# mir-group/allegro

Measured on NVIDIA H100. Metric: atom-steps/sec (energy+forces), higher is better.
Workload: dtype f32

## Files before the change

allegro_b200/_lib.py:

```python
from __future__ import annotations

import ctypes as C
import os
from typing import Optional, Sequence

import torch

from . import build as _build

AB2_F64, AB2_F32, AB2_BF16 = 0, 1, 2
ACT_NONE, ACT_SILU, ACT_MUL_DSILU = 0, 1, 2
EPI_NONE, EPI_MUL_DSILU = 0, 1
NL_SILU, NL_MISH, NL_GELU = 1, 2, 3
NOT_ELIGIBLE = -1
MAX_SEG = 4

DTYPE_ENUM = {torch.float64: AB2_F64, torch.float32: AB2_F32, torch.bfloat16: AB2_BF16}
ACC_DTYPE = {torch.float64: torch.float64, torch.float32: torch.float32, torch.bfloat16: torch.float32}

_LIB: Optional[C.CDLL] = None

_vp, _i64, _i32, _dbl = C.c_void_p, C.c_int64, C.c_int, C.c_double

_SIGNATURES = {
# ... 12 lines not shown
    "ab2_linear_packed_bytes": ([_i32, _i32, _i32], C.c_int64),
    "ab2_linear_pack": ([_i32, _i32, _i32, _vp, _vp, _vp], C.c_int),
    "ab2_mlp2_readout": ([_i32, _i32, _i64, _i32, _i32, _i32, _i32, _vp, _i64, _vp, _i64, _vp, _i64, _vp, _i64, _vp, _i64, _vp, _i64, _vp, _vp, _vp], C.c_int),
    "ab2_mlp2": ([_i32, _i32, _i64, _i32, _i32, _i32, _i32, _vp, _vp, _vp, _vp, _vp, _vp, _vp, _i64, _i32, _vp, _vp, _vp, _vp, _vp], C.c_int),
    "ab2_mlp2_nl": ([_i32, _i32, _i64, _i32, _i32, _i32, _i32, _vp, _vp, _vp, _vp, _vp, _vp, _vp, _i64, _i32, _vp, _vp, _vp, _vp, _vp, _i32], C.c_int),
    "ab2_mlp2_readout_nl": ([_i32, _i32, _i64, _i32, _i32, _i32, _i32, _vp, _i64, _vp, _i64, _vp, _i64, _vp, _i64, _vp, _i64, _vp, _i64, _vp, _vp, _vp, _i32],
                            C.c_int),
    "ab2_env_sum": ([_i32, _i32, _i64, _i32, _vp, _vp, _vp, _i64, _dbl, _vp, _vp], C.c_int),
    "ab2_env_bwd": ([_i32, _i32, _i64, _i64, _i32, _vp, _vp, _vp, _vp, _i64, _vp, _dbl, _vp, _i64, _vp, _vp], C.c_int),
    "ab2_tp_fwd": ([_i32, _i32, _i64, _i64, _i32, _i32, _i32, _i32, _vp, _vp, _vp, _vp, _vp, _vp, _i32, _vp, _vp, _i64, _vp, _vp], C.c_int),
    "ab2_tp_bwd": ([_i32, _i32, _i64, _i64, _i32, _i32, _i32, _i32, _vp, _vp, _vp, _vp, _vp, _vp, _i32, _vp, _vp, _i64, _vp, _vp, _vp, _i64, _vp, _vp, _vp], C.c_int),
    "ab2_tp_chain_fwd": ([_i32, _i32, _i64, _i64, _i32, _vp, _vp, _vp, _vp, _vp, _vp, _vp, _vp, _vp, _vp], C.c_int),
    "ab2_tp_chain_bwd": ([_i32, _i32, _i64, _i64, _i32, _vp, _vp, _vp, _vp, _vp, _vp, _vp, _vp, _vp, _vp, _vp, _vp, _vp, _vp], C.c_int),
    "ab2_edge_sum": ([_i32, _i64, _vp, _vp, _dbl, _vp, _vp], C.c_int),
    "ab2_edge_sum_bwd": ([_i32, _i64, _vp, _vp, _dbl, _vp, _vp], C.c_int),
    "ab2_force_scatter": ([_i32, _i64, _i64, _i64, _vp, _vp, _vp, _vp, _vp, _vp], C.c_int),
    "ab2_force_virial_scatter": ([_i32, _i64, _i64, _i64, _vp, _vp, _vp, _vp, _vp, _vp, _vp, _vp], C.c_int),
    "ab2_transpose_ui": ([_i32, _i64, _i32, _i32, _vp, _vp, _i32, _vp], C.c_int),
    "ab2_edge_vec": ([_i32, _i32, _i64, _vp, _vp, _vp, _vp, _vp, _vp], C.c_int),
    "ab2_radial_fwd": ([_i32, _i64, _i32, _i32, _dbl, _vp, _vp, _vp, _vp, _vp, _i32, _vp, _vp, _vp, _vp, _vp, _vp], C.c_int),
    "ab2_radial_pq_fwd": ([_i32, _i64, _i32, _i32, _dbl, _vp, _vp, _vp, _vp, _vp, _i32, _vp, _vp, _vp, _vp], C.c_int),
    "ab2_radial_pq_bwd": ([_i32, _i64, _i32, _i32, _dbl, _vp, _vp, _vp, _vp, _vp, _i32, _vp, _vp, _vp, _vp, _vp, _vp], C.c_int),
    "ab2_radial_pq_bwd_nl": ([_i32, _i64, _i32, _i32, _dbl, _vp, _vp, _vp, _vp, _vp, _i32, _vp, _vp, _vp, _vp, _vp, _vp, _i32], C.c_int),
    "ab2_zbl": ([_i32, _i64, _i32, _dbl, _dbl, _vp, _vp, _vp, _vp, _vp, _vp, _vp, _vp, _vp], C.c_int),
    "ab2_p2p_mailbox_bytes": ([_i32, _i32], C.c_int64),
    "ab2_p2p_alloc": ([_i64, C.POINTER(C.c_void_p)], C.c_int),
    "ab2_p2p_free": ([_vp], C.c_int),
    "ab2_p2p_get_handle": ([_vp, _vp], C.c_int),
    "ab2_p2p_open_handle": ([_vp, C.POINTER(C.c_void_p)], C.c_int),
    "ab2_p2p_close_handle": ([_vp], C.c_int),
    "ab2_p2p_error": ([_vp, _i32, _i32, _vp], C.c_int),
    "ab2_p2p_begin": ([_vp, _vp], C.c_int),
    "ab2_p2p_push_rows": ([_i32, _i32, _i32, _vp, _vp, _i32, _dbl, _vp, _i32, _i32, _vp, _vp, _vp], C.c_int),
    "ab2_p2p_wait_unpack": ([_i32, _i32, _i32, _vp, _i32, _i32, _vp, _i32, _vp, _vp, _i32, _vp], C.c_int),
    "ab2_p2p_allreduce_energy": ([_vp, _i32, _i32, _i32, _vp, _vp, _vp, _vp, _vp], C.c_int),
    "ab2_p2p_mailbox_bytes_ex": ([_i32, _i32, _i32], C.c_int64),
    "ab2_p2p_push_rows_w": ([_i32, _i32, _vp, _vp, _i32, _vp, _i32, _i32, _vp, _vp, _vp], C.c_int),
    "ab2_p2p_wait_unpack_w": ([_i32, _i32, _vp, _i32, _i32, _vp, _i32, _vp, _vp, _vp, _vp], C.c_int),
    "ab2_p2p_allreduce_vec": ([_vp, _i32, _i32, _i32, _i32, _vp, _vp, _vp, _vp, _vp], C.c_int),
    "ab2_slab_plan_count": ([_i32, _i32, _i64, _vp, _vp, _vp, _i32, _i32, _dbl, _dbl, _dbl, _vp, _vp, _vp], C.c_int),
    "ab2_slab_plan_fill": ([_i64, _vp, _vp, _vp, _vp, _vp, _vp], C.c_int),
    "ab2_nl_bin": ([_i32, _i64, _vp, _vp, _vp, _vp, _vp, _dbl, _vp, _vp], C.c_int),
    "ab2_nl_count": ([_i32, _i64, _vp, _vp, _vp, _vp, _vp, _dbl, _vp, _vp, _vp, _vp], C.c_int),
    "ab2_nl_fill": ([_i32, _i64, _vp, _vp, _vp, _vp, _vp, _dbl, _vp, _vp, _vp, _vp, _vp, _vp], C.c_int),
    "ab2_nl_lattice_bin": ([_i32, _i64, _vp, _vp, _vp, _vp, _vp, _vp, _dbl, _vp, _vp], C.c_int),
    "ab2_nl_lattice_count": ([_i32, _i64, _vp, _vp, _vp, _vp, _vp, _vp, _dbl, _vp, _vp, _vp, _vp], C.c_int),
# ... 584 lines not shown
    counts = torch.empty(n_centres, dtype=torch.int32, device=pos.device)
    with _timed(name + "_count"):
        _check(count_fn(dt, n_centres, _ptr(pos), *geom, _ptr(cell_start), _ptr(order), _ptr(counts), _stream()))
    row_ptr = torch.zeros(n_centres + 1, dtype=torch.int32, device=pos.device)
    row_ptr[1:] = torch.cumsum(counts, 0).to(torch.int32)
    E = int(row_ptr[-1])
    nbr = torch.empty(E, dtype=torch.int32, device=pos.device)
    shift = torch.empty(E, 3, dtype=pos.dtype, device=pos.device)
    if E:
        with _timed(name + "_fill"):
            _check(fill_fn(dt, n_centres, _ptr(pos), *geom, _ptr(cell_start), _ptr(order), _ptr(row_ptr), _ptr(nbr), _ptr(shift), _stream()))
    return row_ptr, nbr, shift


def radial_pq_fwd(dtype, S: int, p_cut: float, vec, ctr, nbr, types, rmax_table, bessel_w, PQ) -> torch.Tensor:
    E = ctr.shape[0]
    out = torch.empty(E, S, dtype=dtype, device=vec.device)
    with _timed("radial_fwd"):
        _check(load().ab2_radial_pq_fwd(DTYPE_ENUM[dtype], E, S, bessel_w.numel(), float(p_cut), _ptr(vec), _ptr(ctr), _ptr(nbr), _ptr(types),
                                        _ptr(rmax_table), rmax_table.shape[0], _ptr(bessel_w), _ptr(_contig(PQ, "PQ")), _ptr(out), _stream()))
    return out


def radial_pq_bwd(dtype, S: int, p_cut: float, vec, ctr, nbr, types, rmax_table, bessel_w, PQ, g_out, aux, gvec, nonlin: int = NL_SILU):
    E = ctr.shape[0]
    args = (DTYPE_ENUM[dtype], E, S, bessel_w.numel(), float(p_cut), _ptr(vec), _ptr(ctr), _ptr(nbr), _ptr(types), _ptr(rmax_table),
            rmax_table.shape[0], _ptr(bessel_w), _ptr(_contig(PQ, "PQ")), _ptr(_contig(g_out, "g_out")),
            _ptr(_contig(aux, "aux")) if aux is not None else None, _ptr(gvec), _stream())
    with _timed("radial_bwd"):
        _check(load().ab2_radial_pq_bwd(*args) if nonlin == NL_SILU else load().ab2_radial_pq_bwd_nl(*args, nonlin))


def _slab_plan(mode: int, pos: torch.Tensor, image: Optional[torch.Tensor], box, rank: int, world: int, width: float, jump: float,
               r_list: float, n_lists: int):
    n = pos.shape[0]
    if n == 0:
        return [torch.empty(0, dtype=torch.int64, device=pos.device) for _ in range(n_lists)], 0
    nblk = (n + 255) // 256
    cls = torch.empty(n, dtype=torch.uint8, device=pos.device)
    counts = torch.empty(nblk, 4, dtype=torch.int32, device=pos.device)
    boxa = (C.c_double * 3)(*[float(b) for b in box])
    with _timed("slab_plan_count"):
        _check(load().ab2_slab_plan_count(DTYPE_ENUM[pos.dtype], mode, n, _ptr(_contig(pos, "pos")), _ptr(image), boxa, int(rank), int(world),
                                          float(width), float(jump), float(r_list), _ptr(cls), _ptr(counts), _stream()))
    incl = torch.cumsum(counts, 0, dtype=torch.int32)
    offsets = (incl - counts).contiguous()
    lists = [torch.empty(n, dtype=torch.int64, device=pos.device) for _ in range(n_lists)]
    ptrs = [_ptr(t) for t in lists] + [None] * (3 - n_lists)
# ... 82 lines not shown
```

allegro_b200/csrc/linear_tc.cu:

```cuda
#include <cuda.h>

#include <type_traits>

#include "common.cuh"

extern int g_ab2_opt_linear_tc;
extern int g_ab2_opt_linear_tma;
extern int g_ab2_opt_tc_debug;

namespace {

constexpr int BM = 128;
constexpr int KC = 32;
constexpr int NSTAGE = 4;
constexpr int RAW_STAGE = 256 * 4 * 16;
constexpr int EPI_LD = 40;
constexpr int NCONS = 8;
constexpr int EPI_BYTES = NCONS * 16 * EPI_LD * 4;
constexpr int STAGE_HALF = BM * KC * 2;
constexpr int NPROD = 8;
constexpr int NTHREADS = (NPROD + NCONS) * 32;
constexpr int MAX_W_BYTES = 128 * 1024;
constexpr int MAX_K = 512;
constexpr int MAX_N = 128;
constexpr int MAX_CHUNK = MAX_N / 32;
constexpr int TAIL_BARS = 2 * NSTAGE * 8, TAIL_CHUNK = MAX_CHUNK * 32, TAIL_KMAP = (MAX_K / 8) * 16;
constexpr int TAIL_BYTES = TAIL_BARS + TAIL_CHUNK + 2 * TAIL_KMAP;
// ... 835 lines not shown
    uint64_t* rbars = reinterpret_cast<uint64_t*>(reinterpret_cast<uint8_t*>(sKseg) + (MAX_K / 32) * 16);
    const uint32_t bar0 = smem_u32(bars), rbar0 = smem_u32(rbars);
    const int nkb = p.K / KC;

    if (threadIdx.x == 0) tma_init_bars(bar0, rbar0, WPG);
    if (threadIdx.x < MAX_K / 32) {
        sKseg[threadIdx.x] = tma_kseg_entry(p, threadIdx.x);
    } else if (threadIdx.x >= 64 && threadIdx.x < 64 + MAX_CHUNK) {
        sChunk[threadIdx.x - 64] = tc_chunk_info<TSrc>(p, (threadIdx.x - 64) * 32);
    }
    stage_w(sW, p.Wpacked, p.Wlo, w_half);
    fence_proxy_async();
    __syncthreads();
    TcCtx ctx;
    ctx.sW = sW; ctx.sA = sA; ctx.sEpi = sEpi; ctx.sChunk = sChunk; ctx.bar0 = bar0;
    ctx.nkb = nkb; ctx.stage_bytes = stage_bytes; ctx.w_half = w_half;
    const int64_t my_tiles = (p.num_tiles > blockIdx.x) ? (p.num_tiles - blockIdx.x + gridDim.x - 1) / gridDim.x : 0;
    const int64_t total = my_tiles * nkb;

    if (warp >= NPROD) {
        tc_consumer_role<TSrc, SPLIT, NCH, NL>(p, ctx, warp - NPROD, lane);
    } else {
        tma_converter_role<G, NL>(p, maps, NR, ctx, sRaw, sKseg, rbar0, total, warp, lane);
    }
}

constexpr int MLP2_MAX_H = 64;
constexpr int MLP2_CHUNK = 64;
constexpr int MLP2_MAX_CHUNKS = 4;
constexpr int MLP2_TAIL = TAIL_BARS + (1 + MLP2_MAX_CHUNKS) * TAIL_CHUNK + (MAX_K / 32) * 16 + 8 * 8;

struct Mlp2Params {
    TcParams s1;
    TcParams s2[MLP2_MAX_CHUNKS];
    int n0[MLP2_MAX_CHUNKS];
    int n2;
    int w2_npad;
    int backward;
    const float* pre;
    int64_t pre_ld;
    const float* gout1;
    int64_t gout1_ld;
    const float* w1row;
};

template <int NCH>
// ... 457 lines not shown
    return fn;
}

static bool tc_make_map(CUtensorMap* map, const void* ptr, int64_t ld, int width, int64_t M) {
    EncodeTiledFn fn = tc_encode_fn();
    if (!fn) return false;
    const cuuint64_t dims[2] = {(cuuint64_t)width, (cuuint64_t)M};
    const cuuint64_t strides[1] = {(cuuint64_t)ld * 4};
    const cuuint32_t box[2] = {(cuuint32_t)KC, (cuuint32_t)BM};
    const cuuint32_t estr[2] = {1, 1};
    return fn(map, CU_TENSOR_MAP_DATA_TYPE_FLOAT32, 2, const_cast<void*>(ptr), dims, strides, box, estr, CU_TENSOR_MAP_INTERLEAVE_NONE,
              CU_TENSOR_MAP_SWIZZLE_128B, CU_TENSOR_MAP_L2_PROMOTION_L2_128B, CU_TENSOR_MAP_FLOAT_OOB_FILL_NONE) == CUDA_SUCCESS;
}

template <typename F>
static int tc_with_nl(int nonlin, F&& f) {
    switch (nonlin) {
        case AB2_NL_MISH: return f(std::integral_constant<int, AB2_NL_MISH>{});
        case AB2_NL_GELU: return f(std::integral_constant<int, AB2_NL_GELU>{});
        default: return f(std::integral_constant<int, AB2_NL_SILU>{});
    }
}

static int tc_launch_tma(TcParams& p, int w_bytes, int stage_bytes, int max_smem, unsigned grid, cudaStream_t st, bool dry, int nonlin) {
    TmaMaps maps;
    memset(&maps, 0, sizeof(maps));
    if (!tc_encode_fn()) return -1;
    for (int s = 0; s < p.n_a && !dry; ++s) {
        if (!tc_make_map(&maps.a[s], p.a[s].ptr, p.a[s].ld, p.a[s].width, p.M)) return -1;
        if (p.a[s].aux && !tc_make_map(&maps.x[s], p.a[s].aux, p.a[s].aux_ld, p.a[s].width, p.M)) return -1;
    }
    const int raw_slot = TMA_BOX_BYTES * (p.has_aux ? 2 : 1);
    const int plans[6][3] = {{4, 8, 4}, {4, 4, 4}, {2, 4, 4}, {2, 2, 4}, {2, 4, 2}, {2, 2, 2}};
    int G = 0, NR = 0, nstage = 0;
    size_t smem = 0;
    for (int q = 0; q < 6 && !G; ++q) {
        const size_t need = 1024 + ((w_bytes + 127) & ~127) + (size_t)plans[q][2] * stage_bytes + EPI_BYTES + TAIL_BYTES +
                            (size_t)plans[q][1] * raw_slot;
        if (need <= (size_t)max_smem) { G = plans[q][0]; NR = plans[q][1]; nstage = plans[q][2]; smem = need; }
    }
    if (!G) return -1;
    if (dry) return 0;
    p.nstage = nstage;
    auto go = [&](auto kern) -> int {
        if (cudaFuncSetAttribute(kern, cudaFuncAttributeMaxDynamicSharedMemorySize, (int)smem) != cudaSuccess) {
            cudaGetLastError();
            return -1;
        }
        kern<<<grid, NTHREADS, smem, st>>>(p, maps, NR);
        return 0;
    };
    return tc_with_nl(nonlin, [&](auto nl) -> int {
        constexpr int NL = decltype(nl)::value;
        switch ((G == 4 ? 4 : 0) + p.Npad / 32) {
            case 1: return go(linear_tma_kernel<2, 1, NL>);
            case 2: return go(linear_tma_kernel<2, 2, NL>);
            case 3: return go(linear_tma_kernel<2, 3, NL>);
            case 4: return go(linear_tma_kernel<2, 4, NL>);
            case 5: return go(linear_tma_kernel<4, 1, NL>);
            case 6: return go(linear_tma_kernel<4, 2, NL>);
            case 7: return go(linear_tma_kernel<4, 3, NL>);
            case 8: return go(linear_tma_kernel<4, 4, NL>);
        }
        return -1;
// ... 112 lines not shown
        const int ns = (N - n0 < width) ? (N - n0) : width;
        void* so_ptr[AB2_MAX_SEG];
        int64_t so_ld[AB2_MAX_SEG];
        int32_t so_w[AB2_MAX_SEG], so_acc[AB2_MAX_SEG];
        int cnt = 0, seg_lo = 0;
        for (int s = 0; s < n_o; ++s) {
            const int seg_hi = seg_lo + o_width[s];
            const int a = n0 > seg_lo ? n0 : seg_lo, b = (n0 + ns) < seg_hi ? (n0 + ns) : seg_hi;
            if (a < b) {
                so_ptr[cnt] = reinterpret_cast<uint8_t*>(o_ptr[s]) + (size_t)(a - seg_lo) * esz;
                so_ld[cnt] = o_ld[s];
                so_w[cnt] = b - a;
                so_acc[cnt] = o_accum ? o_accum[s] : 0;
                ++cnt;
            }
            seg_lo = seg_hi;
        }
        const void* aux_s = aux ? reinterpret_cast<const uint8_t*>(aux) + (size_t)n0 * esz : nullptr;
        const int rc = tc_launch_slice(dtype, M, K, ns, n_a, a_ptr, a_ld, a_width, a_aux, a_aux_ld, act, hi + (size_t)n0 * K * 2,
                                       lo + (size_t)n0 * K * 2, cnt, so_ptr, so_ld, so_w, so_acc, epi, aux_s, aux_ld, st, nonlin);
        if (rc != 0) return n0 == 0 ? -1 : 1;
    }
    return 0;
}

extern "C" int ab2_mlp2_nl(int dtype, int backward, int64_t M, int K, int H, int N, int n_a, const void* const* a_ptr, const int64_t* a_ld,
                           const int32_t* a_width, const void* W1_packed, const void* W2_packed, const void* w1_row, void* pre, int64_t pre_ld,
                           int n_o, void* const* o_ptr, const int64_t* o_ld, const int32_t* o_width, const int32_t* o_accum, void* stream,
                           int nonlin) {
    AB2_CHECK_ARG(nonlin == AB2_NL_SILU || nonlin == AB2_NL_MISH || nonlin == AB2_NL_GELU, "nonlinearity");
    AB2_CHECK_ARG(n_a >= 1 && n_a <= AB2_MAX_SEG && n_o >= 1 && n_o <= AB2_MAX_SEG, "segment count");
    AB2_CHECK_ARG(K > 0 && H > 0 && N > 0 && pre && pre_ld >= H, "shape");
    int ks = 0, ns = 0;
    for (int s = 0; s < n_a; ++s) {
        AB2_CHECK_ARG(a_ptr[s] && a_width[s] > 0 && a_ld[s] >= a_width[s], "A segment");
        ks += a_width[s];
    }
    for (int s = 0; s < n_o; ++s) {
        AB2_CHECK_ARG(o_ptr[s] && o_width[s] > 0 && o_ld[s] >= o_width[s], "output segment");
        ns += o_width[s];
    }
    AB2_CHECK_ARG(ks == K, "A segment widths must sum to K");
    AB2_CHECK_ARG(ns == N, "output segment widths must sum to N");
    const bool rank1 = w1_row != nullptr;
    AB2_CHECK_ARG(!rank1 || (backward && K == 1 && n_a == 1), "rank-1 mode is the backward of a single output column");
    if (M == 0) return 0;
// ... 206 lines not shown
```

allegro_b200/csrc/radial.cu:

```cuda
#include "common.cuh"

#define AB2_MAX_BESSEL 16

template <typename T>
__device__ __forceinline__ T ab2_sin(T x);
template <>
__device__ __forceinline__ float ab2_sin<float>(float x) { return sinf(x); }
template <>
__device__ __forceinline__ double ab2_sin<double>(double x) { return sin(x); }
template <typename T>
__device__ __forceinline__ T ab2_cos(T x);
template <>
__device__ __forceinline__ float ab2_cos<float>(float x) { return cosf(x); }
template <>
__device__ __forceinline__ double ab2_cos<double>(double x) { return cos(x); }
__device__ __forceinline__ float ab2_pow(float x, float p) { return powf(x, p); }
__device__ __forceinline__ double ab2_pow(double x, double p) { return pow(x, p); }

template <typename TPos, typename TAcc>
__global__ void __launch_bounds__(256) edge_vec_kernel(int64_t E, const TPos* __restrict__ pos, const int32_t* __restrict__ ctr,
                                                       const int32_t* __restrict__ nbr, const TPos* __restrict__ shift,
                                                       TAcc* __restrict__ vec) {
    const int64_t z = (int64_t)blockIdx.x * 256 + threadIdx.x;
    if (z >= E) return;
    const int64_t i = ctr[z], j = nbr[z];
#pragma unroll
    for (int a = 0; a < 3; ++a) {
        TPos d = pos[j * 3 + a] - pos[i * 3 + a];
        if (shift) d += shift[z * 3 + a];
        vec[z * 3 + a] = (TAcc)d;
    }
}

template <typename TAcc, bool GRAD>
__device__ __forceinline__ void bessel_basis(TAcc x, TAcc p, int nb, const TAcc* __restrict__ bw, TAcc* B, TAcc* dB) {
    const TAcc PI = TAcc(3.14159265358979323846);
    if (x >= TAcc(1)) {
        for (int n = 0; n < nb; ++n) {
            B[n] = TAcc(0);
            if (GRAD) dB[n] = TAcc(0);
        }
        return;
    }
    const TAcc xp = ab2_pow(x, p);
    const TAcc a = (p + 1) * (p + 2) / 2, b = p * (p + 2), c = p * (p + 1) / 2;
    const TAcc f = TAcc(1) - a * xp + b * xp * x - c * xp * x * x;
    const TAcc df = GRAD ? (-a * p * xp / x + b * (p + 1) * xp - c * (p + 2) * xp * x) : TAcc(0);
    const TAcc inv = TAcc(1) / (PI * x);
    for (int n = 0; n < nb; ++n) {
        const TAcc arg = PI * bw[n] * x;
        const TAcc s = ab2_sin(arg) * inv;
        B[n] = s * f;
        if (GRAD) {
            const TAcc ds = (bw[n] * ab2_cos(arg) - s) / x;
            dB[n] = ds * f + s * df;
        }
    }
}

template <typename TAct, typename TAcc>
__global__ void __launch_bounds__(256) radial_fwd_kernel(int64_t E, int S_rc, int nb, TAcc p, const TAcc* __restrict__ vec,
                                                         const int32_t* __restrict__ ctr, const int32_t* __restrict__ nbr,
                                                         const int32_t* __restrict__ types, const TAcc* __restrict__ rmax_table,
                                                         int num_types, const TAcc* __restrict__ bw, const TAcc* __restrict__ Wb,
                                                         const TAcc* __restrict__ cemb, const TAcc* __restrict__ nemb,
                                                         TAct* __restrict__ e0) {
    __shared__ TAcc sB[AB2_MAX_BESSEL][256];
    __shared__ int s_tc[256], s_tn[256];
    const int t = threadIdx.x;
    const int64_t z0 = (int64_t)blockIdx.x * 256;
    {
        const int64_t z = z0 + t;
        TAcc B[AB2_MAX_BESSEL];
        int tc = 0, tn = 0;
        if (z < E) {
            const TAcc vx = vec[z * 3], vy = vec[z * 3 + 1], vz = vec[z * 3 + 2];
            const TAcc r = sqrt(vx * vx + vy * vy + vz * vz);
            tc = types[ctr[z]];
            tn = types[nbr[z]];
// ... 282 lines not shown
```

allegro_b200/nn/_pipeline.py:

```python
from __future__ import annotations

import math
from typing import Dict, List, Optional

import torch

from .. import _lib
from ..data import EdgeCSR
from ._mlp import PackedMLP


def _env_perm(U: int, n_ir: int, individual: bool = True) -> torch.Tensor:
    r = torch.arange(n_ir).view(-1, 1)
    u = torch.arange(U).view(1, -1)
    if not individual:
        return (u + 0 * r).reshape(-1)
    return (u * n_ir + r).reshape(-1)


class _Saved:
    __slots__ = ("csr", "vec", "Y", "w0", "omega", "V", "gamma", "pre_lat", "pre_read", "X", "fold", "chain")


_BAKED_TABLES = {}
# ... 303 lines not shown
        self.rmax_table = edge_norm.rmax_table.detach().to(device=device, dtype=acc).contiguous()
        self.bessel_w = radial.bessel_encode.bessel_weights.detach().reshape(-1).to(device=device, dtype=acc).contiguous()
        self.Wb = te.basis_linear.folded_weights()[0].to(device=device, dtype=acc).contiguous()
        self.cemb = te.center_embed.weight.detach().to(device=device, dtype=acc).contiguous()
        self.nemb = te.neighbor_embed.weight.detach().to(device=device, dtype=acc).contiguous()
        self.PQ, self.S_pq, self.fold_radial = None, 0, False
        nb = int(self.bessel_w.numel())
        import os as _os

        if nb == 8 and _os.environ.get("ALLEGRO_B200_RADIAL_PQ", "1") == "1":
            Wb64 = te.basis_linear.folded_weights()[0].detach().double().cpu()
            ce, ne = te.center_embed.weight.detach().double().cpu(), te.neighbor_embed.weight.detach().double().cpu()
            T = ce.shape[0]
            temb = torch.cat([ce.unsqueeze(1).expand(T, T, -1), ne.unsqueeze(0).expand(T, T, -1)], dim=-1)
            PQ0 = temb.reshape(T * T, 1, -1) * Wb64.unsqueeze(0)
            if self.mlp.is_two_layer_nonlinear and self.mlp.dims[1] <= 128 and _os.environ.get("ALLEGRO_B200_FOLD_RADIAL", "1") == "1":
                self.fold_radial = True
                PQ0 = PQ0 @ self.mlp.W64[0]
            if PQ0.shape[-1] <= 128:
                self.PQ = PQ0.to(device=device, dtype=acc).contiguous()
                self.S_pq = int(PQ0.shape[-1])
            else:
                self.fold_radial = False

    def forward(self, vec, csr: EdgeCSR, types_i32, outs):
        dt = self.dtype
        if self.kind == "spline":
            from ._spline import spline_forward

            t64 = types_i32.long()
            e0, sp_saved = spline_forward(vec, t64[csr.ctr.long()], t64[csr.nbr.long()], self.rmax64, self.sp_lower, self.sp_upper, self.sp_const,
                                          self.sp_w, self.num_types, dt)
            return ("spline", sp_saved, self.mlp.forward([e0], outs))
        if self.fold_radial:
            h = _lib.radial_pq_fwd(dt, self.S_pq, self.p, vec, csr.ctr, csr.nbr, types_i32, self.rmax_table, self.bessel_w, self.PQ)
            _lib.linear([h], self.mlp.W[1], outs, act=_lib.ACT_SILU, W_packed=self.mlp.Wp[1], **self.mlp.nl_kw)
            return ("pq_fold", None, [h])
        if self.PQ is not None:
            e0 = _lib.radial_pq_fwd(dt, self.S_pq, self.p, vec, csr.ctr, csr.nbr, types_i32, self.rmax_table, self.bessel_w, self.PQ)
        else:
            e0 = _lib.radial_fwd(dt, self.S_rc, self.p, vec, csr.ctr, csr.nbr, types_i32, self.rmax_table, self.bessel_w, self.Wb, self.cemb, self.nemb)
        return ("bessel", None, self.mlp.forward([e0], outs))

    def backward(self, saved, gouts, vec, csr: EdgeCSR, types_i32, gvec):
        kind, sp_saved, pre = saved
        dt = self.dtype
        E = vec.shape[0]
        if kind == "pq_fold":
            g_h = self.mlp.hidden_grad(gouts)
            _lib.radial_pq_bwd(dt, self.S_pq, self.p, vec, csr.ctr, csr.nbr, types_i32, self.rmax_table, self.bessel_w, self.PQ, g_h, pre[0], gvec,
                               **self.mlp.nl_kw)
            return
        g_e0 = torch.empty(E, self.S_rc, dtype=dt, device=vec.device)
        if self.mlp.is_two_layer_nonlinear:
            self.mlp.backward_plain(gouts, pre, [g_e0])
        else:
            self.mlp.backward(gouts, pre, [g_e0], [False])
        if kind == "spline":
            from ._spline import spline_backward

            gvec += spline_backward(sp_saved, g_e0, self.sp_w, self.num_types).to(gvec.dtype)
        elif self.PQ is not None:
            _lib.radial_pq_bwd(dt, self.S_pq, self.p, vec, csr.ctr, csr.nbr, types_i32, self.rmax_table, self.bessel_w, self.PQ, g_e0, None, gvec)
        else:
            _lib.radial_bwd(dt, self.S_rc, self.p, vec, csr.ctr, csr.nbr, types_i32, self.rmax_table, self.bessel_w, self.Wb, self.cemb, self.nemb, g_e0, gvec)


def energy_forces(core: "AllegroCore", up: UpstreamPack, csr: EdgeCSR, pos: torch.Tensor, types_i32: torch.Tensor,
                  shift_vec: Optional[torch.Tensor], gEi_scale: Optional[torch.Tensor], want_virial: bool = False, pair=None,
                  frame_ptr: Optional[torch.Tensor] = None, want_atomic_virial: bool = False):
    dt, acc = core.dtype, core.acc
# ... 65 lines not shown
```

include/allegro_b200.h:

```cpp
#ifndef ALLEGRO_B200_H
#define ALLEGRO_B200_H
#include <stdint.h>

#ifdef __cplusplus
extern "C" {
#endif

enum { AB2_F64 = 0, AB2_F32 = 1, AB2_BF16 = 2 };
enum { AB2_ACT_NONE = 0, AB2_ACT_SILU = 1, AB2_ACT_MUL_DSILU = 2 };
enum { AB2_EPI_NONE = 0, AB2_EPI_MUL_DSILU = 1 };
enum { AB2_NL_SILU = 1, AB2_NL_MISH = 2, AB2_NL_GELU = 3 };

#define AB2_MAX_SEG 4
#define AB2_MAX_LMAX 4

const char* ab2_last_error(void);
int ab2_version(void);
int ab2_device_ok(void);
int ab2_set_option(const char* key, int value);


int ab2_op_scatter_env(int dtype, int64_t E, int64_t row , double sf,
                       const void* x2, const int64_t* idxs, void* gamma, void* stream);

// ... 132 lines not shown
int ab2_nl_frames_fill(int pos_dtype, int64_t n, int64_t n_frames, const int32_t* frame_ptr, const void* pos,
                       const void* cell, const void* inv_cell, const int32_t* pbc, const int32_t* nimg, double r_max,
                       const int32_t* row_ptr, int32_t* nbr, void* shift, void* stream);

int64_t ab2_frame_scratch_elems(int64_t total, int64_t n_frames);
int ab2_frame_sum(int acc_dtype, int64_t n, int64_t n_frames, const int32_t* frame_ptr, const void* x, double* scratch,
                  int64_t scratch_elems, void* out, void* stream);
int ab2_frame_virial(int acc_dtype, int64_t E, int64_t n_frames, const int32_t* frame_ptr, const int32_t* row_ptr,
                     const void* vec, const void* gvec, double* scratch, int64_t scratch_elems, void* W, void* stream);
int ab2_frame_heat_current(int acc_dtype, int64_t n, int64_t n_frames, const int32_t* frame_ptr, const void* e_atom,
                           const void* vel, const void* W, double* scratch, int64_t scratch_elems, void* J, void* stream);

int ab2_radial_pq_fwd(int dtype, int64_t E, int S, int num_bessels, double p_cut, const void* vec,
                      const int32_t* ctr, const int32_t* nbr, const int32_t* types, const void* rmax_table,
                      int num_types, const void* bessel_w, const void* PQ, void* out, void* stream);
int ab2_radial_pq_bwd(int dtype, int64_t E, int S, int num_bessels, double p_cut, const void* vec,
                      const int32_t* ctr, const int32_t* nbr, const int32_t* types, const void* rmax_table,
                      int num_types, const void* bessel_w, const void* PQ, const void* g_out, const void* aux,
                      void* gvec, void* stream);
int ab2_radial_pq_bwd_nl(int dtype, int64_t E, int S, int num_bessels, double p_cut, const void* vec,
                         const int32_t* ctr, const int32_t* nbr, const int32_t* types, const void* rmax_table,
                         int num_types, const void* bessel_w, const void* PQ, const void* g_out, const void* aux,
                         void* gvec, void* stream, int nonlin);

int ab2_zbl(int acc_dtype, int64_t E, int num_types, double p_cut, double qq, const void* vec, const int32_t* ctr,
            const int32_t* nbr, const int32_t* types, const void* Z, const void* rmax_table, void* Ez, void* gvec,
            void* stream);


int64_t ab2_p2p_mailbox_bytes(int max_rows, int world);
int ab2_p2p_alloc(int64_t bytes, void** ptr);
int ab2_p2p_free(void* ptr);
int ab2_p2p_get_handle(void* ptr, void* handle64_host);
int ab2_p2p_open_handle(const void* handle64_host, void** ptr);
int ab2_p2p_close_handle(void* ptr);
int ab2_p2p_error(void* my_mailbox, int max_rows, int world, void* stream);
int ab2_p2p_begin(void* step_counter, void* stream);
int ab2_p2p_push_rows(int src_dtype, int kind, int side, const void* src, const int64_t* idx, int n, double shift_x,
                      void* peer_mailbox, int max_rows, int world, const void* step_counter, void* done_counter,
                      void* stream);
int ab2_p2p_wait_unpack(int dst_dtype, int kind, int side, void* my_mailbox, int max_rows, int world,
                        const void* step_counter, int n, void* dst, const int64_t* idx, int accumulate, void* stream);
int ab2_p2p_allreduce_energy(const void* e_local, int rank, int world, int max_rows, void* const* peers_dev,
                             void* my_mailbox, const void* step_counter, void* e_total, void* stream);

#define AB2_P2P_EXT_VIRIAL 1
// ... 22 lines not shown
```

Before: 3.466 million.

## Fuse radial MLP hidden-grad GEMM with radial basis adjoint in one TMA kernel

Adds a tensor-core TMA kernel that computes the output-layer gradient GEMM (gradient segments times packed W_out) and, in its epilogue, applies the activation derivative, contracts with the Bessel-basis derivative through PQ, and writes the edge-vector gradient. This replaces the separate hidden_grad GEMM plus radial_pq_bwd kernel for f32 with 8 Bessels and S of 32 or 64. The goal is to avoid materialising and re-reading the E x S hidden gradient and to save a launch. In exchange, the consumer warps' epilogue recomputes the Bessel basis and does per-row PQ gathers, which adds register pressure and shared-memory use. The bessel_basis helper moves into a shared header.

```diff
diff --git a/allegro_b200/_lib.py b/allegro_b200/_lib.py
--- a/allegro_b200/_lib.py
+++ b/allegro_b200/_lib.py
@@ -58,6 +58,9 @@
     "ab2_radial_pq_fwd": ([_i32, _i64, _i32, _i32, _dbl, _vp, _vp, _vp, _vp, _vp, _i32, _vp, _vp, _vp, _vp], C.c_int),
     "ab2_radial_pq_bwd": ([_i32, _i64, _i32, _i32, _dbl, _vp, _vp, _vp, _vp, _vp, _i32, _vp, _vp, _vp, _vp, _vp, _vp], C.c_int),
     "ab2_radial_pq_bwd_nl": ([_i32, _i64, _i32, _i32, _dbl, _vp, _vp, _vp, _vp, _vp, _i32, _vp, _vp, _vp, _vp, _vp, _vp, _i32], C.c_int),
+    "ab2_radial_pq_bwd_gemm_plan": ([_i32, _i32, _i32, _i32, _vp], C.c_int),
+    "ab2_radial_pq_bwd_gemm_nl": ([_i32, _i64, _i32, _i32, _dbl, _vp, _vp, _vp, _vp, _vp, _i32, _vp, _vp, _i32, _vp, _vp, _vp, _vp, _vp, _i64, _vp,
+                                   _vp, _i32], C.c_int),
     "ab2_zbl": ([_i32, _i64, _i32, _dbl, _dbl, _vp, _vp, _vp, _vp, _vp, _vp, _vp, _vp, _vp], C.c_int),
     "ab2_p2p_mailbox_bytes": ([_i32, _i32], C.c_int64),
     "ab2_p2p_alloc": ([_i64, C.POINTER(C.c_void_p)], C.c_int),
@@ -688,8 +691,30 @@
     return out
 
 
-def radial_pq_bwd(dtype, S: int, p_cut: float, vec, ctr, nbr, types, rmax_table, bessel_w, PQ, g_out, aux, gvec, nonlin: int = NL_SILU):
+def radial_pq_bwd_gemm_plan(dtype, S: int, num_bessels: int, seg_widths: Sequence[int]) -> bool:
+    w = (C.c_int32 * len(seg_widths))(*seg_widths)
+    return load().ab2_radial_pq_bwd_gemm_plan(DTYPE_ENUM[dtype], int(S), int(num_bessels), len(seg_widths), w) == 0
+
+
+def radial_pq_bwd(dtype, S: int, p_cut: float, vec, ctr, nbr, types, rmax_table, bessel_w, PQ, g_out, aux, gvec, nonlin: int = NL_SILU, *,
+                  W_out: Optional[torch.Tensor] = None, W_out_packed: Optional[torch.Tensor] = None):
     E = ctr.shape[0]
+    if W_out_packed is not None:
+        K, S_w = W_out.shape
+        assert S_w == S and aux is not None and aux.dtype == dtype and tuple(aux.shape) == (E, S)
+        aux, aux_ld = _row_strided(aux, "aux")
+        n = len(g_out)
+        g_ptr, g_ld, g_w = (C.c_void_p * n)(), (C.c_int64 * n)(), (C.c_int32 * n)()
+        for s, t in enumerate(g_out):
+            t, ld = _row_strided(t, f"gradient segment {s}")
+            assert t.dtype == dtype and t.shape[0] == E
+            g_ptr[s], g_ld[s], g_w[s] = _ptr(t).value, ld, t.shape[1]
+        assert sum(g_w) == K
+        with _timed("radial_bwd"):
+            _check(load().ab2_radial_pq_bwd_gemm_nl(DTYPE_ENUM[dtype], E, S, bessel_w.numel(), float(p_cut), _ptr(vec), _ptr(ctr), _ptr(nbr),
+                                                    _ptr(types), _ptr(rmax_table), rmax_table.shape[0], _ptr(bessel_w), _ptr(_contig(PQ, "PQ")),
+                                                    n, g_ptr, g_ld, g_w, _ptr(W_out_packed), _ptr(aux), aux_ld, _ptr(gvec), _stream(), nonlin))
+        return
     args = (DTYPE_ENUM[dtype], E, S, bessel_w.numel(), float(p_cut), _ptr(vec), _ptr(ctr), _ptr(nbr), _ptr(types), _ptr(rmax_table),
             rmax_table.shape[0], _ptr(bessel_w), _ptr(_contig(PQ, "PQ")), _ptr(_contig(g_out, "g_out")),
             _ptr(_contig(aux, "aux")) if aux is not None else None, _ptr(gvec), _stream())
diff --git a/allegro_b200/csrc/linear_tc.cu b/allegro_b200/csrc/linear_tc.cu
--- a/allegro_b200/csrc/linear_tc.cu
+++ b/allegro_b200/csrc/linear_tc.cu
@@ -3,6 +3,7 @@
 #include <type_traits>
 
 #include "common.cuh"
+#include "radial_basis.cuh"
 
 extern int g_ab2_opt_linear_tc;
 extern int g_ab2_opt_linear_tma;
@@ -884,6 +885,178 @@
         tc_consumer_role<TSrc, SPLIT, NCH, NL>(p, ctx, warp - NPROD, lane);
     } else {
         tma_converter_role<G, NL>(p, maps, NR, ctx, sRaw, sKseg, rbar0, total, warp, lane);
+    }
+}
+
+struct RadialAdj {
+    const float* vec;
+    const int32_t* ctr;
+    const int32_t* nbr;
+    const int32_t* types;
+    const float* rmax_table;
+    const float* bw;
+    const float* PQ;
+    const float* h;
+    float* gvec;
+    int64_t h_ld;
+    int num_types;
+    float p_cut;
+};
+
+constexpr int RADJ_LD = 16;
+
+__device__ __forceinline__ float2 ldg64_nc(const float* p) {
+    float2 v;
+    asm volatile("ld.global.nc.v2.f32 {%0, %1}, [%2];" : "=f"(v.x), "=f"(v.y) : "l"(p));
+    return v;
+}
+
+__device__ __forceinline__ int radj_rows(const TcParams& p, int64_t m_base) {
+    const int64_t left64 = p.M - m_base;
+    return left64 >= 16 ? 16 : (left64 > 0 ? (int)left64 : 0);
+}
+
+template <int NCH>
+__device__ __forceinline__ void radial_adjoint_prologue(const TcParams& p, const RadialAdj& ra, float* stg, float2 (&hv)[2][4 * NCH],
+                                                        int64_t m_base, int lane) {
+    const int rows_left = radj_rows(p, m_base);
+    if (rows_left == 0) return;
+    const int ra0 = lane >> 2, q = lane & 3;
+#pragma unroll
+    for (int hr = 0; hr < 2; ++hr) {
+        const int r = min(ra0 + 8 * hr, rows_left - 1);
+        const float* hz = ra.h + (m_base + r) * ra.h_ld + 2 * q;
+#pragma unroll
+        for (int j = 0; j < 4 * NCH; ++j) hv[hr][j] = ldg64_nc(hz + 8 * j);
+    }
+    const int row = lane & 15, half = lane >> 4;
+    float* s = stg + row * RADJ_LD;
+    float B[4], dB[4];
+    float vx = 0.f, vy = 0.f, vz = 0.f, den = 1.f, g0 = 0.f, g1 = 0.f, g2 = 0.f;
+    int pair = 0;
+    if (row < rows_left) {
+        const int64_t z = m_base + row;
+        vx = ra.vec[z * 3]; vy = ra.vec[z * 3 + 1]; vz = ra.vec[z * 3 + 2];
+        if (!half) { g0 = ra.gvec[z * 3]; g1 = ra.gvec[z * 3 + 1]; g2 = ra.gvec[z * 3 + 2]; }
+        const float r = sqrt(vx * vx + vy * vy + vz * vz);
+        pair = ra.types[ra.ctr[z]] * ra.num_types + ra.types[ra.nbr[z]];
+        const float rmax = ra.rmax_table[pair];
+        bessel_basis<float, true>(r / rmax, ra.p_cut, 4, ra.bw + 4 * half, B, dB);
+        den = rmax * r;
+    } else {
+#pragma unroll
+        for (int n = 0; n < 4; ++n) dB[n] = 0.f;
+    }
+#pragma unroll
+    for (int n = 0; n < 4; ++n) s[4 * half + n] = dB[n];
+    if (!half) {
+        s[8] = __int_as_float(pair); s[9] = den; s[10] = vx; s[11] = vy; s[12] = vz;
+        s[13] = g0; s[14] = g1; s[15] = g2;
+    }
+}
+
+template <int NCH, int NL>
+__device__ __forceinline__ void radial_adjoint_epilogue(const TcParams& p, const RadialAdj& ra, float* stg, const float (&acc)[16 * NCH],
+                                                        const float2 (&hv)[2][4 * NCH], int64_t m_base, int lane) {
+    constexpr int S = 32 * NCH;
+    const int rows_left = radj_rows(p, m_base);
+    if (rows_left == 0) return;
+    __syncwarp();
+    const int ra0 = lane >> 2, q = lane & 3;
+    const float* sa = stg + ra0 * RADJ_LD;
+    const float* sb = stg + (ra0 + 8) * RADJ_LD;
+    float dBa[8], dBb[8];
+#pragma unroll
+    for (int n = 0; n < 8; ++n) { dBa[n] = sa[n]; dBb[n] = sb[n]; }
+    const int pa = __float_as_int(sa[8]), pb = __float_as_int(sb[8]);
+    const float* ma = ra.PQ + (int64_t)pa * 8 * S + 2 * q;
+    const float* mb = ra.PQ + (int64_t)pb * 8 * S + 2 * q;
+    const bool same = pa == pb;
+    float ga = 0.f, gb = 0.f;
+#pragma unroll
+    for (int j = 0; j < 4 * NCH; ++j) {
+        float sa0 = 0.f, sa1 = 0.f, sb0 = 0.f, sb1 = 0.f;
+#pragma unroll
+        for (int n = 0; n < 8; ++n) {
+            const float2 wa = __ldg(reinterpret_cast<const float2*>(ma + n * S + 8 * j));
+            const float2 wb = same ? wa : __ldg(reinterpret_cast<const float2*>(mb + n * S + 8 * j));
+            sa0 += dBa[n] * wa.x;
+            sa1 += dBa[n] * wa.y;
+            sb0 += dBb[n] * wb.x;
+            sb1 += dBb[n] * wb.y;
+        }
+        float a0 = acc[4 * j], a1 = acc[4 * j + 1], b0 = acc[4 * j + 2], b1 = acc[4 * j + 3];
+        a0 *= dact_f<NL>(hv[0][j].x);
+        a1 *= dact_f<NL>(hv[0][j].y);
+        b0 *= dact_f<NL>(hv[1][j].x);
+        b1 *= dact_f<NL>(hv[1][j].y);
+        ga += a0 * sa0;
+        ga += a1 * sa1;
+        gb += b0 * sb0;
+        gb += b1 * sb1;
+    }
+    ga += __shfl_xor_sync(0xffffffffu, ga, 1);
+    ga += __shfl_xor_sync(0xffffffffu, ga, 2);
+    gb += __shfl_xor_sync(0xffffffffu, gb, 1);
+    gb += __shfl_xor_sync(0xffffffffu, gb, 2);
+    if (q < 2) {
+        const int r = ra0 + 8 * q;
+        if (r < rows_left) {
+            const float* s = q ? sb : sa;
+            const float f = (q ? gb : ga) / s[9];
+            float* gv = ra.gvec + (m_base + r) * 3;
+            gv[0] = s[13] + f * s[10];
+            gv[1] = s[14] + f * s[11];
+            gv[2] = s[15] + f * s[12];
+        }
+    }
+    __syncwarp();
+}
+
+template <int G, int NCH, int NL>
+__global__ void __launch_bounds__(NTHREADS, 1) radial_adjoint_tma_kernel(const TcParams p, const __grid_constant__ TmaMaps maps, int NR,
+                                                                       const RadialAdj ra) {
+    constexpr int WPG = NPROD / G;
+    extern __shared__ __align__(1024) uint8_t smem[];
+    const int warp = __shfl_sync(0xffffffffu, threadIdx.x >> 5, 0), lane = threadIdx.x & 31;
+    const int w_half = p.Npad * p.K * 2;
+    const int w_bytes = 2 * w_half;
+    const int stage_bytes = 2 * STAGE_HALF;
+    uint8_t* sRaw = smem + ((1024u - (smem_u32(smem) & 1023u)) & 1023u);
+    uint8_t* sW = sRaw + (size_t)NR * TMA_BOX_BYTES;
+    uint8_t* sA = sW + ((w_bytes + 127) & ~127);
+    float* sEpi = reinterpret_cast<float*>(sA + p.nstage * stage_bytes);
+    uint64_t* bars = reinterpret_cast<uint64_t*>(reinterpret_cast<uint8_t*>(sEpi) + EPI_BYTES);
+    int4* sKseg = reinterpret_cast<int4*>(reinterpret_cast<uint8_t*>(bars) + TAIL_BARS + TAIL_CHUNK);
+    uint64_t* rbars = reinterpret_cast<uint64_t*>(reinterpret_cast<uint8_t*>(sKseg) + (MAX_K / 32) * 16);
+    const uint32_t bar0 = smem_u32(bars), rbar0 = smem_u32(rbars);
+    const int nkb = p.K / KC;
+
+    if (threadIdx.x == 0) tma_init_bars(bar0, rbar0, WPG);
+    if (threadIdx.x < MAX_K / 32) sKseg[threadIdx.x] = tma_kseg_entry(p, threadIdx.x);
+    stage_w(sW, p.Wpacked, p.Wlo, w_half);
+    fence_proxy_async();
+    __syncthreads();
+    TcCtx ctx;
+    ctx.sW = sW; ctx.sA = sA; ctx.sEpi = sEpi; ctx.sChunk = nullptr; ctx.bar0 = bar0;
+    ctx.nkb = nkb; ctx.stage_bytes = stage_bytes; ctx.w_half = w_half;
+    const int64_t my_tiles = (p.num_tiles > blockIdx.x) ? (p.num_tiles - blockIdx.x + gridDim.x - 1) / gridDim.x : 0;
+
+    if (warp >= NPROD) {
+        const int cw = warp - NPROD, wg = cw >> 2, w4 = cw & 3;
+        float* stg = sEpi + cw * 16 * EPI_LD;
+        int stage = 0;
+        uint32_t phase = 0;
+        float acc[16 * NCH];
+        float2 hv[2][4 * NCH];
+        for (int64_t tile = blockIdx.x; tile < p.num_tiles; tile += gridDim.x) {
+            const int64_t m_base = tile * BM + wg * 64 + w4 * 16;
+            radial_adjoint_prologue<NCH>(p, ra, stg, hv, m_base, lane);
+            tc_mma_ring<true, NCH>(acc, p, ctx, wg, lane, stage, phase);
+            radial_adjoint_epilogue<NCH, NL>(p, ra, stg, acc, hv, m_base, lane);
+        }
+    } else {
+        tma_converter_role<G, NL>(p, maps, NR, ctx, sRaw, sKseg, rbar0, my_tiles * nkb, warp, lane);
     }
 }
 
@@ -1387,6 +1560,18 @@
     }
 }
 
+static bool tc_tma_plan(int w_bytes, int stage_bytes, int raw_slot, int max_smem, int& G, int& NR, int& nstage, size_t& smem) {
+    const int plans[6][3] = {{4, 8, 4}, {4, 4, 4}, {2, 4, 4}, {2, 2, 4}, {2, 4, 2}, {2, 2, 2}};
+    G = NR = nstage = 0;
+    smem = 0;
+    for (int q = 0; q < 6 && !G; ++q) {
+        const size_t need = 1024 + ((w_bytes + 127) & ~127) + (size_t)plans[q][2] * stage_bytes + EPI_BYTES + TAIL_BYTES +
+                            (size_t)plans[q][1] * raw_slot;
+        if (need <= (size_t)max_smem) { G = plans[q][0]; NR = plans[q][1]; nstage = plans[q][2]; smem = need; }
+    }
+    return G != 0;
+}
+
 static int tc_launch_tma(TcParams& p, int w_bytes, int stage_bytes, int max_smem, unsigned grid, cudaStream_t st, bool dry, int nonlin) {
     TmaMaps maps;
     memset(&maps, 0, sizeof(maps));
@@ -1396,15 +1581,9 @@
         if (p.a[s].aux && !tc_make_map(&maps.x[s], p.a[s].aux, p.a[s].aux_ld, p.a[s].width, p.M)) return -1;
     }
     const int raw_slot = TMA_BOX_BYTES * (p.has_aux ? 2 : 1);
-    const int plans[6][3] = {{4, 8, 4}, {4, 4, 4}, {2, 4, 4}, {2, 2, 4}, {2, 4, 2}, {2, 2, 2}};
     int G = 0, NR = 0, nstage = 0;
     size_t smem = 0;
-    for (int q = 0; q < 6 && !G; ++q) {
-        const size_t need = 1024 + ((w_bytes + 127) & ~127) + (size_t)plans[q][2] * stage_bytes + EPI_BYTES + TAIL_BYTES +
-                            (size_t)plans[q][1] * raw_slot;
-        if (need <= (size_t)max_smem) { G = plans[q][0]; NR = plans[q][1]; nstage = plans[q][2]; smem = need; }
-    }
-    if (!G) return -1;
+    if (!tc_tma_plan(w_bytes, stage_bytes, raw_slot, max_smem, G, NR, nstage, smem)) return -1;
     if (dry) return 0;
     p.nstage = nstage;
     auto go = [&](auto kern) -> int {
@@ -1563,6 +1742,78 @@
         if (rc != 0) return n0 == 0 ? -1 : 1;
     }
     return 0;
+}
+
+static int radj_plan(int dtype, int S, int num_bessels, int n_seg, const int32_t* seg_width, int& K, int& G, int& NR, int& nstage, size_t& smem) {
+    if (dtype != AB2_F32 || num_bessels != 8 || (S != 32 && S != 64) || n_seg < 1 || n_seg > AB2_MAX_SEG || !seg_width) return AB2_NOT_ELIGIBLE;
+    K = 0;
+    for (int s = 0; s < n_seg; ++s) {
+        if (seg_width[s] <= 0 || seg_width[s] % KC != 0) return AB2_NOT_ELIGIBLE;
+        K += seg_width[s];
+    }
+    if (K > MAX_K || !tc_encode_fn()) return AB2_NOT_ELIGIBLE;
+    int num_sms = 0, max_smem = 0;
+    tc_device_limits(num_sms, max_smem);
+    return tc_tma_plan(S * K * 2 * 2, 2 * STAGE_HALF, TMA_BOX_BYTES, max_smem, G, NR, nstage, smem) ? 0 : AB2_NOT_ELIGIBLE;
+}
+
+extern "C" int ab2_radial_pq_bwd_gemm_plan(int dtype, int S, int num_bessels, int n_seg, const int32_t* seg_width) {
+    int K, G, NR, nstage;
+    size_t smem;
+    return radj_plan(dtype, S, num_bessels, n_seg, seg_width, K, G, NR, nstage, smem);
+}
+
+extern "C" int ab2_radial_pq_bwd_gemm_nl(int dtype, int64_t E, int S, int num_bessels, double p_cut, const void* vec, const int32_t* ctr,
+                                         const int32_t* nbr, const int32_t* types, const void* rmax_table, int num_types, const void* bessel_w,
+                                         const void* PQ, int n_seg, const void* const* g_ptr, const int64_t* g_ld, const int32_t* g_width,
+                                         const void* W_packed, const void* aux, int64_t aux_ld, void* gvec, void* stream, int nonlin) {
+    AB2_CHECK_ARG(nonlin == AB2_NL_SILU || nonlin == AB2_NL_MISH || nonlin == AB2_NL_GELU, "nonlinearity");
+    int K = 0, G = 0, NR = 0, nstage = 0;
+    size_t smem = 0;
+    AB2_CHECK_ARG(radj_plan(dtype, S, num_bessels, n_seg, g_width, K, G, NR, nstage, smem) == 0,
+                  "radial_pq_bwd_gemm: shape not taken (see ab2_radial_pq_bwd_gemm_plan)");
+    if (E == 0) return 0;
+    AB2_CHECK_ARG(vec && ctr && nbr && types && rmax_table && bessel_w && PQ && g_ptr && g_ld && W_packed && aux && gvec, "null pointer");
+    AB2_CHECK_ARG(E < ((int64_t)1 << 31), "radial_pq_bwd_gemm: E >= 2^31");
+    AB2_CHECK_ARG(!(reinterpret_cast<uintptr_t>(aux) & 7) && aux_ld % 2 == 0 && aux_ld >= S, "radial_pq_bwd_gemm: aux rows must be 8-byte aligned");
+    for (int s = 0; s < n_seg; ++s)
+        AB2_CHECK_ARG(g_ptr[s] && !(reinterpret_cast<uintptr_t>(g_ptr[s]) & 15) && (g_ld[s] * 4) % 16 == 0,
+                      "radial_pq_bwd_gemm: gradient segments must be 16-byte aligned");
+    int num_sms = 0, max_smem = 0;
+    tc_device_limits(num_sms, max_smem);
+    TcParams p;
+    memset(&p, 0, sizeof(p));
+    p.M = E; p.K = K; p.N = S; p.Npad = S; p.n_a = n_seg; p.act = AB2_ACT_NONE; p.epi = AB2_EPI_NONE;
+    p.Wpacked = W_packed;
+    p.Wlo = reinterpret_cast<const uint8_t*>(W_packed) + (size_t)S * K * 2;
+    p.num_tiles = (E + BM - 1) / BM;
+    p.nstage = nstage;
+    for (int s = 0; s < n_seg; ++s) { p.a[s].ptr = g_ptr[s]; p.a[s].ld = g_ld[s]; p.a[s].width = g_width[s]; }
+    TmaMaps maps;
+    memset(&maps, 0, sizeof(maps));
+    for (int s = 0; s < n_seg; ++s) AB2_CHECK_ARG(tc_make_map(&maps.a[s], g_ptr[s], g_ld[s], g_width[s], E), "radial_pq_bwd_gemm: tensor map");
+    RadialAdj ra;
+    ra.vec = (const float*)vec; ra.ctr = ctr; ra.nbr = nbr; ra.types = types; ra.rmax_table = (const float*)rmax_table;
+    ra.bw = (const float*)bessel_w; ra.PQ = (const float*)PQ; ra.h = (const float*)aux; ra.gvec = (float*)gvec; ra.h_ld = aux_ld;
+    ra.num_types = num_types; ra.p_cut = (float)p_cut;
+    const unsigned grid = (unsigned)((p.num_tiles < num_sms) ? p.num_tiles : num_sms);
+    cudaStream_t st = (cudaStream_t)stream;
+    auto go = [&](auto kern) -> int {
+        AB2_CHECK_ARG(cudaFuncSetAttribute(kern, cudaFuncAttributeMaxDynamicSharedMemorySize, (int)smem) == cudaSuccess,
+                      "radial_pq_bwd_gemm: shared-memory plan");
+        kern<<<grid, NTHREADS, smem, st>>>(p, maps, NR, ra);
+        AB2_CUDA_LAUNCH_CHECK();
+        return 0;
+    };
+    return tc_with_nl(nonlin, [&](auto nl) -> int {
+        constexpr int NL = decltype(nl)::value;
+        switch ((G == 4 ? 2 : 0) + S / 32) {
+            case 1: return go(radial_adjoint_tma_kernel<2, 1, NL>);
+            case 2: return go(radial_adjoint_tma_kernel<2, 2, NL>);
+            case 3: return go(radial_adjoint_tma_kernel<4, 1, NL>);
+            default: return go(radial_adjoint_tma_kernel<4, 2, NL>);
+        }
+    });
 }
 
 extern "C" int ab2_mlp2_nl(int dtype, int backward, int64_t M, int K, int H, int N, int n_a, const void* const* a_ptr, const int64_t* a_ld,
diff --git a/allegro_b200/csrc/radial.cu b/allegro_b200/csrc/radial.cu
--- a/allegro_b200/csrc/radial.cu
+++ b/allegro_b200/csrc/radial.cu
@@ -1,21 +1,7 @@
 #include "common.cuh"
+#include "radial_basis.cuh"
 
 #define AB2_MAX_BESSEL 16
-
-template <typename T>
-__device__ __forceinline__ T ab2_sin(T x);
-template <>
-__device__ __forceinline__ float ab2_sin<float>(float x) { return sinf(x); }
-template <>
-__device__ __forceinline__ double ab2_sin<double>(double x) { return sin(x); }
-template <typename T>
-__device__ __forceinline__ T ab2_cos(T x);
-template <>
-__device__ __forceinline__ float ab2_cos<float>(float x) { return cosf(x); }
-template <>
-__device__ __forceinline__ double ab2_cos<double>(double x) { return cos(x); }
-__device__ __forceinline__ float ab2_pow(float x, float p) { return powf(x, p); }
-__device__ __forceinline__ double ab2_pow(double x, double p) { return pow(x, p); }
 
 template <typename TPos, typename TAcc>
 __global__ void __launch_bounds__(256) edge_vec_kernel(int64_t E, const TPos* __restrict__ pos, const int32_t* __restrict__ ctr,
@@ -29,32 +15,6 @@
         TPos d = pos[j * 3 + a] - pos[i * 3 + a];
         if (shift) d += shift[z * 3 + a];
         vec[z * 3 + a] = (TAcc)d;
-    }
-}
-
-template <typename TAcc, bool GRAD>
-__device__ __forceinline__ void bessel_basis(TAcc x, TAcc p, int nb, const TAcc* __restrict__ bw, TAcc* B, TAcc* dB) {
-    const TAcc PI = TAcc(3.14159265358979323846);
-    if (x >= TAcc(1)) {
-        for (int n = 0; n < nb; ++n) {
-            B[n] = TAcc(0);
-            if (GRAD) dB[n] = TAcc(0);
-        }
-        return;
-    }
-    const TAcc xp = ab2_pow(x, p);
-    const TAcc a = (p + 1) * (p + 2) / 2, b = p * (p + 2), c = p * (p + 1) / 2;
-    const TAcc f = TAcc(1) - a * xp + b * xp * x - c * xp * x * x;
-    const TAcc df = GRAD ? (-a * p * xp / x + b * (p + 1) * xp - c * (p + 2) * xp * x) : TAcc(0);
-    const TAcc inv = TAcc(1) / (PI * x);
-    for (int n = 0; n < nb; ++n) {
-        const TAcc arg = PI * bw[n] * x;
-        const TAcc s = ab2_sin(arg) * inv;
-        B[n] = s * f;
-        if (GRAD) {
-            const TAcc ds = (bw[n] * ab2_cos(arg) - s) / x;
-            dB[n] = ds * f + s * df;
-        }
     }
 }
 
diff --git a/allegro_b200/csrc/radial_basis.cuh b/allegro_b200/csrc/radial_basis.cuh
--- /dev/null
+++ b/allegro_b200/csrc/radial_basis.cuh
@@ -0,0 +1,44 @@
+#pragma once
+
+#include "common.cuh"
+
+template <typename T>
+__device__ __forceinline__ T ab2_sin(T x);
+template <>
+__device__ __forceinline__ float ab2_sin<float>(float x) { return sinf(x); }
+template <>
+__device__ __forceinline__ double ab2_sin<double>(double x) { return sin(x); }
+template <typename T>
+__device__ __forceinline__ T ab2_cos(T x);
+template <>
+__device__ __forceinline__ float ab2_cos<float>(float x) { return cosf(x); }
+template <>
+__device__ __forceinline__ double ab2_cos<double>(double x) { return cos(x); }
+__device__ __forceinline__ float ab2_pow(float x, float p) { return powf(x, p); }
+__device__ __forceinline__ double ab2_pow(double x, double p) { return pow(x, p); }
+
+template <typename TAcc, bool GRAD>
+__device__ __forceinline__ void bessel_basis(TAcc x, TAcc p, int nb, const TAcc* __restrict__ bw, TAcc* B, TAcc* dB) {
+    const TAcc PI = TAcc(3.14159265358979323846);
+    if (x >= TAcc(1)) {
+        for (int n = 0; n < nb; ++n) {
+            B[n] = TAcc(0);
+            if (GRAD) dB[n] = TAcc(0);
+        }
+        return;
+    }
+    const TAcc xp = ab2_pow(x, p);
+    const TAcc a = (p + 1) * (p + 2) / 2, b = p * (p + 2), c = p * (p + 1) / 2;
+    const TAcc f = TAcc(1) - a * xp + b * xp * x - c * xp * x * x;
+    const TAcc df = GRAD ? (-a * p * xp / x + b * (p + 1) * xp - c * (p + 2) * xp * x) : TAcc(0);
+    const TAcc inv = TAcc(1) / (PI * x);
+    for (int n = 0; n < nb; ++n) {
+        const TAcc arg = PI * bw[n] * x;
+        const TAcc s = ab2_sin(arg) * inv;
+        B[n] = s * f;
+        if (GRAD) {
+            const TAcc ds = (bw[n] * ab2_cos(arg) - s) / x;
+            dB[n] = ds * f + s * df;
+        }
+    }
+}
diff --git a/allegro_b200/nn/_pipeline.py b/allegro_b200/nn/_pipeline.py
--- a/allegro_b200/nn/_pipeline.py
+++ b/allegro_b200/nn/_pipeline.py
@@ -349,6 +349,10 @@
                 self.S_pq = int(PQ0.shape[-1])
             else:
                 self.fold_radial = False
+        self.bwd_gemm = False
+        if self.fold_radial and self.mlp.WTp[1] is not None:
+            widths = [fold_embed_of.nw, fold_embed_of.S, fold_embed_of.nw] if self.fold else [self.mlp.dims[-1]]
+            self.bwd_gemm = _lib.radial_pq_bwd_gemm_plan(dtype, self.S_pq, nb, widths)
 
     def forward(self, vec, csr: EdgeCSR, types_i32, outs):
         dt = self.dtype
@@ -374,6 +378,10 @@
         dt = self.dtype
         E = vec.shape[0]
         if kind == "pq_fold":
+            if self.bwd_gemm:
+                _lib.radial_pq_bwd(dt, self.S_pq, self.p, vec, csr.ctr, csr.nbr, types_i32, self.rmax_table, self.bessel_w, self.PQ, list(gouts), pre[0],
+                                   gvec, **self.mlp.nl_kw, W_out=self.mlp.WT[1], W_out_packed=self.mlp.WTp[1])
+                return
             g_h = self.mlp.hidden_grad(gouts)
             _lib.radial_pq_bwd(dt, self.S_pq, self.p, vec, csr.ctr, csr.nbr, types_i32, self.rmax_table, self.bessel_w, self.PQ, g_h, pre[0], gvec,
                                **self.mlp.nl_kw)
diff --git a/include/allegro_b200.h b/include/allegro_b200.h
--- a/include/allegro_b200.h
+++ b/include/allegro_b200.h
@@ -178,6 +178,12 @@
                          const int32_t* ctr, const int32_t* nbr, const int32_t* types, const void* rmax_table,
                          int num_types, const void* bessel_w, const void* PQ, const void* g_out, const void* aux,
                          void* gvec, void* stream, int nonlin);
+int ab2_radial_pq_bwd_gemm_plan(int dtype, int S, int num_bessels, int n_seg, const int32_t* seg_width);
+int ab2_radial_pq_bwd_gemm_nl(int dtype, int64_t E, int S, int num_bessels, double p_cut, const void* vec,
+                              const int32_t* ctr, const int32_t* nbr, const int32_t* types, const void* rmax_table,
+                              int num_types, const void* bessel_w, const void* PQ, int n_seg, const void* const* g_ptr,
+                              const int64_t* g_ld, const int32_t* g_width, const void* W_out_packed, const void* aux,
+                              int64_t aux_ld, void* gvec, void* stream, int nonlin);
 
 int ab2_zbl(int acc_dtype, int64_t E, int num_types, double p_cut, double qq, const void* vec, const int32_t* ctr,
             const int32_t* nbr, const int32_t* types, const void* Z, const void* rmax_table, void* Ez, void* gvec,
```

Result: no change. 3.488 million, median of 6 (+0.6%).
